# fcogidi/X3D-tf

Measured on AMD Instinct MI355X. Metric: clips/sec (fwd+bwd) X3D-M 16x224^2; depthwise HBM GB/s, higher is better.
Workload: dtype bf16

## Files before the change

### x3d-tf_amd/csrc/pw_bwd_wst.hip

```cpp
#include <stdlib.h>

#include "pw_gemm_ws.h"

struct PwBwdWstArgs {
  const void* g; const void* yraw; const float* coef;
  const void* wp; int wp_rows;
  void* dx;
  const void* braw; const float* b_ss; const float* egate; double* nc_sums;
  float* dw;
  int N, Co, Ci;
  long long P;
  int tiles_per_block;
  BnBwdFold fold;
  float* slab;
  int hot;
  int noflush;
};

#define BW_YRP 40

template <typename H, int NW, int KS, int CT>
__global__ __launch_bounds__(512, 2) void pw_bwd_wst_kernel(const PwBwdWstArgs a) {
  typedef typename HV<H>::x8 hx8;
  extern __shared__ __attribute__((aligned(16))) unsigned char smem_raw[];
  typedef H T;
  constexpr int BN = 32, OP = WS_OP, NT = 512, Kp = KS * 16, WP = Kp + 8, CoP = CT * 32, YRP = BW_YRP;
  static_assert(CoP >= Kp, "the row-read copy covers every staged dY row");
  constexpr int NSV = (Kp * 4 + NT - 1) / NT;
  H* Yt = (H*)smem_raw;
  H* Yr = (H*)(smem_raw + (size_t)2 * Kp * 64);
  H* Xh = (H*)(smem_raw + (size_t)2 * Kp * 64 + (size_t)2 * CoP * YRP * 2);
  float* Cs = (float*)(smem_raw + (size_t)2 * Kp * 64 + (size_t)2 * CoP * YRP * 2 + (size_t)NW * 32 * YRP * 2);
  float* Os = Cs + Kp * 4;
  const int tid = threadIdx.x, lane = tid & 63, wid = tid >> 6;
  const int r = lane & 31, half = lane >> 5;
  const int mt = (a.Ci + 31) >> 5;
  const int tiles_per_n = (int)((a.P + BN - 1) / BN);
  const int total_tiles = tiles_per_n * a.N;
  const int tile_begin = blockIdx.x * a.tiles_per_block;
  const int tile_end = min(tile_begin + a.tiles_per_block, total_tiles);
  if (tile_begin >= tile_end) return;
  float* myOs = Os + wid * 32 * OP;
  const int rb = blockIdx.y * NW + wid;
  const bool mw = wid < NW && rb < mt;

  {
    hx8 z;
#pragma unroll
    for (int e = 0; e < 8; e++) z[e] = (H)0.f;
    for (int i = tid; i < 2 * CoP * YRP / 8; i += NT) ((hx8*)Yr)[i] = z;
    for (int k = tid; k < Kp; k += NT) {
      f32x4 c = {0.f, 0.f, 0.f, 0.f};
      if (k < a.Co) {
        float cA_, cB_, cC_;
        bn_bwd_coef_load(a.coef, a.fold, k, blockIdx.x == 0 && blockIdx.y == 0, cA_, cB_, cC_);
        c[0] = cA_; c[1] = cB_; c[2] = cC_;
      }
      *(f32x4*)&Cs[k * 4] = c;
    }
  }

  hx8 A[KS];
  if (mw) {
    const H* wt = (const H*)a.wp + (long long)a.wp_rows * WP + ((long long)rb * KS * 64 + lane) * 8;
#pragma unroll
    for (int ks = 0; ks < KS; ks++) A[ks] = *(const hx8*)(wt + ks * 512);
  } else {
#pragma unroll
    for (int ks = 0; ks < KS; ks++)
#pragma unroll
      for (int e = 0; e < 8; e++) A[ks][e] = (H)0.f;
  }

  hx8 g0[NSV], y0[NSV], g1[NSV], y1[NSV];
  auto issue_loads = [&](int tile_, hx8 (&gr)[NSV], hx8 (&yr)[NSV]) {
    const int tile = a.hot ? tile_begin : min(tile_, tile_end - 1);
    const int n = tile / tiles_per_n;
    const long long p0 = (long long)(tile - n * tiles_per_n) * BN;
#pragma unroll
    for (int i = 0; i < NSV; i++) {
      const int v = tid + i * NT;
      const int k = v >> 2;
      const long long p = p0 + (v & 3) * 8;
      const bool ok = k < a.Co && p < a.P;
      const long long o = ok ? ((long long)n * a.Co + k) * a.P + p : 0;
      gr[i] = *(const hx8*)((const T*)a.g + o);
      yr[i] = *(const hx8*)((const T*)a.yraw + o);
    }
  };
  auto commit = [&](int tile, int buf, const hx8 (&gr)[NSV], const hx8 (&yr)[NSV]) {
    const int n = tile / tiles_per_n;
    const long long p0 = (long long)(tile - n * tiles_per_n) * BN;
#pragma unroll
    for (int i = 0; i < NSV; i++) {
      const int v = tid + i * NT;
      const int k = v >> 2;
      if (k >= Kp) continue;
      const bool ok = k < a.Co && p0 + (v & 3) * 8 < a.P;
      const f32x4 cf = *(const f32x4*)&Cs[k * 4];
      float val[8];
#pragma unroll
      for (int e = 0; e < 8; e++) val[e] = ok ? cf[0] * (float)gr[i][e] + cf[1] * (float)yr[i][e] + cf[2] : 0.f;
      hx8 hv;
#pragma unroll
      for (int e = 0; e < 8; e++) hv[e] = (H)val[e];
      *(hx8*)&Yt[(buf * Kp + k) * BN + (v & 3) * 8] = hv;
      *(hx8*)&Yr[(buf * CoP + k) * YRP + (v & 3) * 8] = hv;
    }
  };

  const int row = lane >> 1, c0 = 16 * (lane & 1);
  const int m = rb * 32 + row;
  const bool mrow = mw && m < a.Ci;
  hx8 eb0[2], eb1[2];
  float gl0, gl1;
  const float* gsrc = a.egate ? a.egate : a.b_ss;
  auto issue_braw = [&](int tile_, hx8 (&eb)[2], float& gl) {
    const int tile = a.hot ? tile_begin : min(tile_, tile_end - 1);
    const int n = tile / tiles_per_n;
    const long long p0 = (long long)(tile - n * tiles_per_n) * BN;
    gl = gsrc[(a.egate && mrow) ? (long long)n * a.Ci + m : 0];
#pragma unroll
    for (int hv = 0; hv < 2; hv++) {
      const long long p = p0 + c0 + 8 * hv;
      const long long o = (mrow && p < a.P) ? ((long long)n * a.Ci + m) * a.P + p : 0;
      eb[hv] = *(const hx8*)((const T*)a.braw + o);
    }
  };

  float st1 = 0.f, st2 = 0.f;
  auto flush_sums = [&](int n) {
    const float s1 = st1 + dpp_get<0xB1, 0xF>(st1), s2 = st2 + dpp_get<0xB1, 0xF>(st2);
    if (mrow && (lane & 1) == 0) {
      double* d = a.nc_sums + ((long long)n * a.Ci + m) * 2;
      atomic_add_d(d, (double)s1);
      atomic_add_d(d + 1, (double)s2);
    }
    st1 = 0.f;
    st2 = 0.f;
  };
  const float sb = mrow ? a.b_ss[m * 2] : 0.f, tb = mrow ? a.b_ss[m * 2 + 1] : 0.f;

  f32x16 acc_dw[CT];
#pragma unroll
  for (int s = 0; s < CT; s++)
#pragma unroll
    for (int e = 0; e < 16; e++) acc_dw[s][e] = 0.f;

  const int g16 = lane >> 4, q = (lane & 15) >> 2, pp = lane & 3;
  const int tr_off = (8 * (g16 >> 1) + q) * BN + 16 * (g16 & 1) + 4 * pp;
  typedef s16x4 __attribute__((address_space(3))) * lds_s16x4_ptr;

  int n_prev = tile_begin / tiles_per_n;
  issue_loads(tile_begin, g0, y0);
  issue_braw(tile_begin, eb0, gl0);
  __syncthreads();
  commit(tile_begin, 0, g0, y0);
  __syncthreads();
  issue_loads(tile_begin + 1, g1, y1);
  issue_loads(tile_begin + 2, g0, y0);

  typedef __attribute__((ext_vector_type(4))) unsigned int u32x4_;
  auto step = [&](int tile, int cur, hx8 (&gr)[NSV], hx8 (&yr)[NSV], hx8 (&eb)[2], float gl, hx8 (&ebn)[2], float& gln) {
    const int n = tile / tiles_per_n;
    const long long p0 = (long long)(tile - n * tiles_per_n) * BN;
    if (n != n_prev) flush_sums(n_prev);
    n_prev = n;
    issue_braw(tile + 1, ebn, gln);
    const float gt = (mrow && a.egate) ? gl : 1.0f;
    __amdgpu_buffer_rsrc_t dxr = __builtin_amdgcn_make_buffer_rsrc((T*)a.dx + (long long)n * a.Ci * a.P, 0,
                                                                   (int)((long long)a.Ci * a.P * 2), 0x00020000);

    f32x16 acc;
#pragma unroll
    for (int e = 0; e < 16; e++) acc[e] = 0.f;
    if (mw) {
      const H* xb = Yt + cur * (Kp * BN) + tr_off;
#pragma unroll
      for (int ks = 0; ks < KS; ks++) {
        const s16x4 b0 = __builtin_amdgcn_ds_read_tr16_b64_v4i16((lds_s16x4_ptr)(xb + ks * 16 * BN));
        const s16x4 b1 = __builtin_amdgcn_ds_read_tr16_b64_v4i16((lds_s16x4_ptr)(xb + (ks * 16 + 4) * BN));
        const s16x8 bs = {b0[0], b0[1], b0[2], b0[3], b1[0], b1[1], b1[2], b1[3]};
        acc = mfma16<H>(A[ks], __builtin_bit_cast(hx8, bs), acc);
      }
    }

    if (tile + 1 < tile_end) commit(tile + 1, cur ^ 1, gr, yr);

    if (mw) {
#pragma unroll
      for (int e = 0; e < 16; e++) myOs[((e & 3) + 8 * (e >> 2) + 4 * half) * OP + r] = acc[e];
#pragma unroll
      for (int hv = 0; hv < 2; hv++) {
        const long long p = p0 + c0 + 8 * hv;
        const bool ok = mrow && p < a.P;
        float val[8];
        {
          const f32x4 v0 = *(const f32x4*)&myOs[row * OP + c0 + 8 * hv], v1 = *(const f32x4*)&myOs[row * OP + c0 + 8 * hv + 4];
#pragma unroll
          for (int e = 0; e < 4; e++) { val[e] = v0[e]; val[4 + e] = v1[e]; }
        }
        hx8 xh;
        const SwishCoef sc_ = swish_coef(sb, tb, gt);
#pragma unroll
        for (int e = 0; e < 8; e++) {
          const float b = (float)eb[hv][e];
          float xs, d_;
          swish_bwd_(sc_, b, xs, d_);
          xh[e] = ok ? (H)xs : (H)0.f;
          const float dv = val[e] * d_;
          val[e] = dv;
          if (ok) { st1 += dv; st2 += dv * b; }
        }
        *(hx8*)&Xh[(wid * 32 + row) * YRP + c0 + 8 * hv] = xh;
        hx8 ov;
#pragma unroll
        for (int e = 0; e < 8; e++) ov[e] = (H)val[e];
        __builtin_amdgcn_raw_buffer_store_b128(__builtin_bit_cast(u32x4_, ov), dxr,
                                               ok ? (unsigned)(((long long)m * a.P + p) * 2) : 0x80000000u, 0, 0);
      }
      const H* yrow = Yr + (cur * CoP + r) * YRP + 8 * half;
      const H* xrow = Xh + (wid * 32 + r) * YRP + 8 * half;
#pragma unroll
      for (int ks = 0; ks < BN / 16; ks++) {
        const hx8 bf = *(const hx8*)(xrow + ks * 16);
#pragma unroll
        for (int s = 0; s < CT; s++) {
          const hx8 af = *(const hx8*)(yrow + s * 32 * YRP + ks * 16);
          acc_dw[s] = mfma16<H>(af, bf, acc_dw[s]);
        }
      }
    }
    __syncthreads();
    issue_loads(tile + 3, gr, yr);
  };
  for (int tile = tile_begin; tile < tile_end; tile += 2) {
    step(tile, 0, g1, y1, eb0, gl0, eb1, gl1);
    if (tile + 1 < tile_end) step(tile + 1, 1, g0, y0, eb1, gl1, eb0, gl0);
  }
  flush_sums(n_prev);

  if (mw && !a.noflush) {
    const int ci = rb * 32 + r;
    float* slab = a.slab ? a.slab + (long long)blockIdx.x * a.Co * a.Ci : nullptr;
#pragma unroll
    for (int s = 0; s < CT; s++)
#pragma unroll
      for (int e = 0; e < 16; e++) {
        const int co = s * 32 + (e & 3) + 8 * (e >> 2) + 4 * half;
        if (co < a.Co && ci < a.Ci) {
          if (slab) slab[(long long)co * a.Ci + ci] = acc_dw[s][e];
          else atomicAdd(&a.dw[(long long)co * a.Ci + ci], acc_dw[s][e]);
        }
      }
  }
}

template <int NW, int KS, int CT>
static inline size_t bw_lds_bytes() {
  return (size_t)2 * KS * 16 * 64 + (size_t)2 * CT * 32 * BW_YRP * 2 + (size_t)NW * 32 * BW_YRP * 2 + (size_t)KS * 16 * 16 +
         (size_t)NW * 32 * WS_OP * 4;
}

bool pw_bwd_wst_applies(const x3d_pw_bwd_args* b) {
  if (x3d_env_int("X3D_PW_BWD_WST", 1) == 0) return false;
  if (!x3d_is_half(b->dtype) || !b->w_panel || (!b->coef && !b->coef_fold) || !b->yraw || b->epi != X3D_EPI_SWISH_BWD || b->tail_c) return false;
  const int ks = (b->Cout + 15) >> 4;
  if (!((b->Cin > 128 && b->Cin <= 224 && ks == 6) || (b->Cin > 224 && b->Cin <= 448 && ks == 12 && x3d_env_int("X3D_PW_BWD_WST5", 1) != 0))) return false;
  const long long P = (long long)b->T * b->H * b->W;
  if (P % 8 || P >= (1ll << 31) || (long long)b->Cin * P * 2 >= (1ll << 31)) return false;
  const void* ps[] = {b->g, b->yraw, b->dx, b->w_panel, b->braw};
  for (const void* p : ps) if (!p || ((uintptr_t)p % 16)) return false;
  return true;
}

static inline void bw_grid(int N, long long P, int Ci, long long* tpb, long long* gx, int* slices) {
  *slices = ceil_div(ceil_div(Ci, 32), 7);
  x3d_persistent_grid(ceil_div_ll(P, 32) * N, x3d_device_cus() / *slices, tpb, gx);
}

template <typename H, int KS, int CT>
static int bw_launch(PwBwdWstArgs& a, hipStream_t st) {
  constexpr int NW = 7;
  const size_t lds = bw_lds_bytes<NW, KS, CT>();
  X3D_DESCRIBE("pw_bwd_wst_kernel<%s, %d, %d, %d>", HV<H>::name, NW, KS, CT);
  auto kern = pw_bwd_wst_kernel<H, NW, KS, CT>;
  static bool attr_set = false;
  if (!attr_set) {
    (void)hipFuncSetAttribute((const void*)kern, hipFuncAttributeMaxDynamicSharedMemorySize, 128 * 1024);
    attr_set = true;
  }
  const long long total_tiles = ceil_div_ll(a.P, 32) * a.N;
  X3D_REQUIRE(total_tiles < (1ll << 31), "pw_bwd_wst: too many tiles");
  long long tpb, gx;
  int slices;
  bw_grid(a.N, a.P, a.Ci, &tpb, &gx, &slices);
  a.tiles_per_block = (int)tpb;
  a.noflush = x3d_env_int("X3D_PW_BWD_NOFLUSH", 0);
  a.hot = x3d_env_int("X3D_PW_BWD_HOT", 0);
  hipLaunchKernelGGL(kern, dim3((unsigned)gx, (unsigned)slices), dim3(512), lds, st, a);
  X3D_LAUNCH_CHECK("pw_bwd_wst");
  return X3D_OK;
}

int pw_bwd_wst(const x3d_pw_bwd_args* b, hipStream_t st) {
  X3D_REQUIRE(b->braw && b->b_scale_shift && b->nc_sums, "pw_bwd: SWISH_BWD needs braw/b_scale_shift/nc_sums");
  PwBwdWstArgs a;
  memset(&a, 0, sizeof(a));
  a.g = b->g; a.yraw = b->yraw; a.coef = b->coef;
  a.wp = b->w_panel; a.wp_rows = (b->Cin + 31) & ~31;
  a.dx = b->dx; a.braw = b->braw; a.b_ss = b->b_scale_shift; a.egate = b->gate; a.nc_sums = b->nc_sums;
  a.dw = b->dw; a.slab = b->dw_slab; a.fold = bn_bwd_fold_arg(b->coef_fold);
  a.N = b->N; a.Co = b->Cout; a.Ci = b->Cin;
  a.P = (long long)b->T * b->H * b->W;
  if (((b->Cout + 15) >> 4) == 12) return b->dtype == X3D_F16 ? bw_launch<f16, 12, 6>(a, st) : bw_launch<bf16, 12, 6>(a, st);
  return b->dtype == X3D_F16 ? bw_launch<f16, 6, 3>(a, st) : bw_launch<bf16, 6, 3>(a, st);
}

int pw_bwd_wst_dw_parts(const x3d_pw_bwd_args* b) {
  long long tpb, gx;
  int slices;
  bw_grid(b->N, (long long)b->T * b->H * b->W, b->Cin, &tpb, &gx, &slices);
  return (int)gx;
}
```

### x3d-tf_amd/csrc/pw_bwd_wsta.hip

```cpp
#include <stdlib.h>

#include "pw_gemm_ws.h"

struct PwBwdWstaArgs {
  const void* g; const void* yraw; const float* coef;
  const void* wp; int wp_rows;
  void* dx;
  const void* add;
  const void* x;
  float* dw;
  const void* tail_c; const void* tail_r; double* tail_sums_c; double* tail_sums_r;
  int N, Co, Ci;
  long long P;
  int tiles_per_block;
  BnBwdFold fold;
  float* slab;
  int hot;
  int noflush;
};

#define BWA_RP 40

template <typename H, int NW, int KS, int CT, int TAIL>
__global__ __launch_bounds__(512, 2) void pw_bwd_wsta_kernel(const PwBwdWstaArgs a) {
  typedef typename HV<H>::x8 hx8;
  extern __shared__ __attribute__((aligned(16))) unsigned char smem_raw[];
  typedef H T;
  constexpr int BN = 32, OP = WS_OP, NT = 512, Kp = KS * 16, WP = Kp + 8, CoP = CT * 32, CiP = NW * 32, RP = BWA_RP;
  static_assert(CoP >= Kp && CT <= 8, "dY rows / weight-gradient waves");
  constexpr int NSV = (Kp * 4 + NT - 1) / NT;
  constexpr size_t YT_B = (size_t)2 * Kp * 64, YR_B = (size_t)2 * CoP * RP * 2, XR_B = (size_t)2 * CiP * RP * 2;
  H* Yt = (H*)smem_raw;
  H* Yr = (H*)(smem_raw + YT_B);
  H* Xr = (H*)(smem_raw + YT_B + YR_B);
  float* Cs = (float*)(smem_raw + YT_B + YR_B + XR_B);
  float* Os = Cs + Kp * 4;
  const int tid = threadIdx.x, lane = tid & 63, wid = tid >> 6;
  const int r = lane & 31, half = lane >> 5;
  const int tiles_per_n = (int)((a.P + BN - 1) / BN);
  const int total_tiles = tiles_per_n * a.N;
  const int tile_begin = blockIdx.x * a.tiles_per_block;
  const int tile_end = min(tile_begin + a.tiles_per_block, total_tiles);
  if (tile_begin >= tile_end) return;
  float* myOs = Os + (wid < NW ? wid : 0) * 32 * OP;
  const bool xw = wid < NW && wid * 32 < a.Ci;
  const bool ww = wid < CT && wid * 32 < a.Co;

  {
    hx8 z;
#pragma unroll
    for (int e = 0; e < 8; e++) z[e] = (H)0.f;
    for (int i = tid; i < (int)((YR_B + XR_B) / 16); i += NT) ((hx8*)Yr)[i] = z;
    for (int k = tid; k < Kp; k += NT) {
      f32x4 c = {0.f, 0.f, 0.f, 0.f};
      if (k < a.Co) {
        float cA_, cB_, cC_;
        bn_bwd_coef_load(a.coef, a.fold, k, blockIdx.x == 0 && blockIdx.y == 0, cA_, cB_, cC_);
        c[0] = cA_; c[1] = cB_; c[2] = cC_;
      }
      *(f32x4*)&Cs[k * 4] = c;
    }
  }

  hx8 A[KS];
  if (xw) {
    const H* wt = (const H*)a.wp + (long long)a.wp_rows * WP + ((long long)wid * KS * 64 + lane) * 8;
#pragma unroll
    for (int ks = 0; ks < KS; ks++) A[ks] = *(const hx8*)(wt + ks * 512);
  } else {
#pragma unroll
    for (int ks = 0; ks < KS; ks++)
#pragma unroll
      for (int e = 0; e < 8; e++) A[ks][e] = (H)0.f;
  }

  hx8 g0[NSV], y0[NSV], g1[NSV], y1[NSV], x0, x1;
  auto issue_loads = [&](int tile_, hx8 (&gr)[NSV], hx8 (&yr)[NSV], hx8& xr) __attribute__((always_inline)) {
    const int tile = a.hot ? tile_begin : min(tile_, tile_end - 1);
    const int n = tile / tiles_per_n;
    const long long p0 = (long long)(tile - n * tiles_per_n) * BN;
#pragma unroll
    for (int i = 0; i < NSV; i++) {
      const int v = tid + i * NT;
      const int k = v >> 2;
      const long long p = p0 + (v & 3) * 8;
      const long long o = (k < a.Co && p < a.P) ? ((long long)n * a.Co + k) * a.P + p : 0;
      gr[i] = *(const hx8*)((const T*)a.g + o);
      yr[i] = *(const hx8*)((const T*)a.yraw + o);
    }
    {
      const int mrow = tid >> 2;
      const long long p = p0 + (tid & 3) * 8;
      const long long o = (mrow < a.Ci && p < a.P) ? ((long long)n * a.Ci + mrow) * a.P + p : 0;
      xr = *(const hx8*)((const T*)a.x + o);
    }
  };
  auto commit = [&](int tile, int buf, const hx8 (&gr)[NSV], const hx8 (&yr)[NSV], const hx8& xr) __attribute__((always_inline)) {
    const int n = tile / tiles_per_n;
    const long long p0 = (long long)(tile - n * tiles_per_n) * BN;
#pragma unroll
    for (int i = 0; i < NSV; i++) {
      const int v = tid + i * NT;
      const int k = v >> 2;
      if (k >= Kp) continue;
      const bool ok = k < a.Co && p0 + (v & 3) * 8 < a.P;
      const f32x4 cf = *(const f32x4*)&Cs[k * 4];
      hx8 hv;
#pragma unroll
      for (int e = 0; e < 8; e++) hv[e] = (H)(ok ? cf[0] * (float)gr[i][e] + cf[1] * (float)yr[i][e] + cf[2] : 0.f);
      *(hx8*)&Yt[(buf * Kp + k) * BN + (v & 3) * 8] = hv;
      *(hx8*)&Yr[(buf * CoP + k) * RP + (v & 3) * 8] = hv;
    }
    const int mrow = tid >> 2;
    if (mrow < CiP) {
      const bool ok = mrow < a.Ci && p0 + (tid & 3) * 8 < a.P;
      hx8 hv = xr;
      if (!ok) {
#pragma unroll
        for (int e = 0; e < 8; e++) hv[e] = (H)0.f;
      }
      *(hx8*)&Xr[(buf * CiP + mrow) * RP + (tid & 3) * 8] = hv;
    }
  };

  const int row = lane >> 1, c0 = 16 * (lane & 1);
  const int m = wid * 32 + row;
  const bool mrow_ok = xw && m < a.Ci;
  constexpr int NEO = 1 + (TAIL >= 1) + (TAIL == 2);
  hx8 eo0[NEO][2], eo1[NEO][2];
  auto issue_epi = [&](int tile_, hx8 (&eo)[NEO][2]) __attribute__((always_inline)) {
    const int tile = a.hot ? tile_begin : min(tile_, tile_end - 1);
    const int n = tile / tiles_per_n;
    const long long p0 = (long long)(tile - n * tiles_per_n) * BN;
#pragma unroll
    for (int hv = 0; hv < 2; hv++) {
      const long long p = p0 + c0 + 8 * hv;
      const long long o = (mrow_ok && p < a.P) ? ((long long)n * a.Ci + m) * a.P + p : 0;
      eo[0][hv] = *(const hx8*)((const T*)a.add + o);
      if constexpr (TAIL >= 1) eo[1][hv] = *(const hx8*)((const T*)a.tail_c + o);
      if constexpr (TAIL == 2) eo[2][hv] = *(const hx8*)((const T*)a.tail_r + o);
    }
  };
  float tg = 0.f, tgc = 0.f, tgr = 0.f;

  f32x16 acc_dw[NW];
#pragma unroll
  for (int s = 0; s < NW; s++)
#pragma unroll
    for (int e = 0; e < 16; e++) acc_dw[s][e] = 0.f;

  const int g16 = lane >> 4, q = (lane & 15) >> 2, pp = lane & 3;
  const int tr_off = (8 * (g16 >> 1) + q) * BN + 16 * (g16 & 1) + 4 * pp;
  typedef s16x4 __attribute__((address_space(3))) * lds_s16x4_ptr;
  typedef __attribute__((ext_vector_type(4))) unsigned int u32x4_;

  issue_loads(tile_begin, g0, y0, x0);
  issue_epi(tile_begin, eo0);
  __syncthreads();
  commit(tile_begin, 0, g0, y0, x0);
  __syncthreads();
  issue_loads(tile_begin + 1, g1, y1, x1);
  issue_loads(tile_begin + 2, g0, y0, x0);

  auto step = [&](int tile, int cur, hx8 (&gr)[NSV], hx8 (&yr)[NSV], hx8& xr, hx8 (&eo)[NEO][2], hx8 (&eon)[NEO][2])
      __attribute__((always_inline)) {
    const int n = tile / tiles_per_n;
    const long long p0 = (long long)(tile - n * tiles_per_n) * BN;
    issue_epi(tile + 1, eon);
    __amdgpu_buffer_rsrc_t dxr = __builtin_amdgcn_make_buffer_rsrc((T*)a.dx + (long long)n * a.Ci * a.P, 0,
                                                                   (int)((long long)a.Ci * a.P * 2), 0x00020000);
    f32x16 acc;
#pragma unroll
    for (int e = 0; e < 16; e++) acc[e] = 0.f;
    if (xw) {
      const H* xb = Yt + cur * (Kp * BN) + tr_off;
#pragma unroll
      for (int ks = 0; ks < KS; ks++) {
        const s16x4 b0 = __builtin_amdgcn_ds_read_tr16_b64_v4i16((lds_s16x4_ptr)(xb + ks * 16 * BN));
        const s16x4 b1 = __builtin_amdgcn_ds_read_tr16_b64_v4i16((lds_s16x4_ptr)(xb + (ks * 16 + 4) * BN));
        const s16x8 bs = {b0[0], b0[1], b0[2], b0[3], b1[0], b1[1], b1[2], b1[3]};
        acc = mfma16<H>(A[ks], __builtin_bit_cast(hx8, bs), acc);
      }
    }
    if (ww) {
      const H* yrow = Yr + (cur * CoP + wid * 32 + r) * RP + 8 * half;
      const H* xrow = Xr + (cur * CiP + r) * RP + 8 * half;
#pragma unroll
      for (int ks = 0; ks < BN / 16; ks++) {
        const hx8 af = *(const hx8*)(yrow + ks * 16);
#pragma unroll
        for (int s = 0; s < NW; s++) {
          const hx8 bf = *(const hx8*)(xrow + s * 32 * RP + ks * 16);
          acc_dw[s] = mfma16<H>(af, bf, acc_dw[s]);
        }
      }
    }
    if (tile + 1 < tile_end) commit(tile + 1, cur ^ 1, gr, yr, xr);

    if (xw) {
#pragma unroll
      for (int e = 0; e < 16; e++) myOs[((e & 3) + 8 * (e >> 2) + 4 * half) * OP + r] = acc[e];
#pragma unroll
      for (int hv = 0; hv < 2; hv++) {
        const long long p = p0 + c0 + 8 * hv;
        const bool ok = mrow_ok && p < a.P;
        float val[8];
        {
          const f32x4 v0 = *(const f32x4*)&myOs[row * OP + c0 + 8 * hv], v1 = *(const f32x4*)&myOs[row * OP + c0 + 8 * hv + 4];
#pragma unroll
          for (int e = 0; e < 4; e++) { val[e] = v0[e]; val[4 + e] = v1[e]; }
        }
#pragma unroll
        for (int e = 0; e < 8; e++) val[e] += (float)eo[0][hv][e];
        if constexpr (TAIL >= 1) {
          const hx8 xv = *(const hx8*)&Xr[(cur * CiP + m) * RP + c0 + 8 * hv];
#pragma unroll
          for (int e = 0; e < 8; e++) {
            const float gm = (ok && (float)xv[e] > 0.f) ? round_to<T>(val[e]) : 0.f;
            val[e] = gm;
            tg += gm;
            tgc += gm * (float)eo[1][hv][e];
            if constexpr (TAIL == 2) tgr += gm * (float)eo[2][hv][e];
          }
        }
        hx8 ov;
#pragma unroll
        for (int e = 0; e < 8; e++) ov[e] = (H)val[e];
        __builtin_amdgcn_raw_buffer_store_b128(__builtin_bit_cast(u32x4_, ov), dxr,
                                               ok ? (unsigned)(((long long)m * a.P + p) * 2) : 0x80000000u, 0, 0);
      }
    }
    __syncthreads();
    issue_loads(tile + 3, gr, yr, xr);
  };
  for (int tile = tile_begin; tile < tile_end; tile += 2) {
    step(tile, 0, g1, y1, x1, eo0, eo1);
    if (tile + 1 < tile_end) step(tile + 1, 1, g0, y0, x0, eo1, eo0);
  }

  if constexpr (TAIL >= 1) {
    const float s0 = tg + dpp_get<0xB1, 0xF>(tg), s1 = tgc + dpp_get<0xB1, 0xF>(tgc);
    float s2 = 0.f;
    if constexpr (TAIL == 2) s2 = tgr + dpp_get<0xB1, 0xF>(tgr);
    if (mrow_ok && (lane & 1) == 0) {
      atomic_add_d(&a.tail_sums_c[m * 2], (double)s0);
      atomic_add_d(&a.tail_sums_c[m * 2 + 1], (double)s1);
      if constexpr (TAIL == 2) {
        atomic_add_d(&a.tail_sums_r[m * 2], (double)s0);
        atomic_add_d(&a.tail_sums_r[m * 2 + 1], (double)s2);
      }
    }
  }
  if (ww && !a.noflush) {
    float* slab = a.slab ? a.slab + (long long)blockIdx.x * a.Co * a.Ci : nullptr;
#pragma unroll
    for (int s = 0; s < NW; s++) {
      const int ci = s * 32 + r;
#pragma unroll
      for (int e = 0; e < 16; e++) {
        const int co = wid * 32 + (e & 3) + 8 * (e >> 2) + 4 * half;
        if (co < a.Co && ci < a.Ci) {
          if (slab) slab[(long long)co * a.Ci + ci] = acc_dw[s][e];
          else atomicAdd(&a.dw[(long long)co * a.Ci + ci], acc_dw[s][e]);
        }
      }
    }
  }
}

template <int NW, int KS, int CT>
static inline size_t bwa_lds_bytes() {
  return (size_t)2 * KS * 16 * 64 + (size_t)2 * CT * 32 * BWA_RP * 2 + (size_t)2 * NW * 32 * BWA_RP * 2 + (size_t)KS * 16 * 16 +
         (size_t)NW * 32 * WS_OP * 4;
}

bool pw_bwd_wsta_applies(const x3d_pw_bwd_args* b) {
  if (x3d_env_int("X3D_PW_BWD_WSTA", 1) == 0) return false;
  if (!x3d_is_half(b->dtype) || !b->w_panel || (!b->coef && !b->coef_fold) || !b->yraw || b->epi != X3D_EPI_ADD || !b->x || !b->add) return false;
  if (b->Cin <= 64 || b->Cin > 96 || ((b->Cout + 15) >> 4) != 14) return false;
  const long long P = (long long)b->T * b->H * b->W;
  if (P % 8 || P >= (1ll << 31) || (long long)b->Cin * P * 2 >= (1ll << 31)) return false;
  const void* ps[] = {b->g, b->yraw, b->dx, b->w_panel, b->x, b->add};
  for (const void* p : ps) if (!p || ((uintptr_t)p % 16)) return false;
  if (b->tail_r) return false;
  if (b->tail_c && ((uintptr_t)b->tail_c % 16)) return false;
  return true;
}

template <typename H, int TAIL>
static int bwa_launch(PwBwdWstaArgs& a, hipStream_t st) {
  constexpr int NW = 3, KS = 14, CT = 7;
  const size_t lds = bwa_lds_bytes<NW, KS, CT>();
  X3D_DESCRIBE("pw_bwd_wsta_kernel<%s, %d, %d, %d, %d>", HV<H>::name, NW, KS, CT, TAIL);
  auto kern = pw_bwd_wsta_kernel<H, NW, KS, CT, TAIL>;
  static bool attr_set = false;
  if (!attr_set) {
    (void)hipFuncSetAttribute((const void*)kern, hipFuncAttributeMaxDynamicSharedMemorySize, 128 * 1024);
    attr_set = true;
  }
  const long long total_tiles = ceil_div_ll(a.P, 32) * a.N;
  X3D_REQUIRE(total_tiles < (1ll << 31), "pw_bwd_wsta: too many tiles");
  long long tpb, gx;
  x3d_persistent_grid(total_tiles, x3d_device_cus(), &tpb, &gx);
  a.tiles_per_block = (int)tpb;
  a.noflush = x3d_env_int("X3D_PW_BWD_NOFLUSH", 0);
  a.hot = x3d_env_int("X3D_PW_BWD_HOT", 0);
  hipLaunchKernelGGL(kern, dim3((unsigned)gx), dim3(512), lds, st, a);
  X3D_LAUNCH_CHECK("pw_bwd_wsta");
  return X3D_OK;
}

int pw_bwd_wsta(const x3d_pw_bwd_args* b, hipStream_t st) {
  X3D_REQUIRE(!b->tail_c || x3d_describe.out || (b->tail_sums_c && (!b->tail_r || b->tail_sums_r)), "pw_bwd: tail_c / tail_r need their sums");
  PwBwdWstaArgs a;
  memset(&a, 0, sizeof(a));
  a.g = b->g; a.yraw = b->yraw; a.coef = b->coef;
  a.wp = b->w_panel; a.wp_rows = (b->Cin + 31) & ~31;
  a.dx = b->dx; a.add = b->add; a.x = b->x; a.dw = b->dw; a.slab = b->dw_slab; a.fold = bn_bwd_fold_arg(b->coef_fold);
  a.tail_c = b->tail_c; a.tail_r = b->tail_r; a.tail_sums_c = b->tail_sums_c; a.tail_sums_r = b->tail_sums_r;
  a.N = b->N; a.Co = b->Cout; a.Ci = b->Cin;
  a.P = (long long)b->T * b->H * b->W;
  const bool tail = b->tail_c != nullptr;
  if (b->dtype == X3D_F16) return tail ? bwa_launch<f16, 1>(a, st) : bwa_launch<f16, 0>(a, st);
  return tail ? bwa_launch<bf16, 1>(a, st) : bwa_launch<bf16, 0>(a, st);
}

int pw_bwd_wsta_dw_parts(const x3d_pw_bwd_args* b) {
  long long tpb, gx;
  x3d_persistent_grid(ceil_div_ll((long long)b->T * b->H * b->W, 32) * b->N, x3d_device_cus(), &tpb, &gx);
  return (int)gx;
}
```

### x3d-tf_amd/csrc/pw_gemm_ws.h

```cpp
#pragma once
#include <type_traits>

#include "pw_gemm_bf16.h"

#define WS_BN 32
#define WS_G 8
#define WS_OP 36
#define WS_MAXMT 4
#ifndef WS_OCC
#define WS_OCC 2
#endif

template <typename H, int PRO, int EPI>
__global__ __launch_bounds__(256, WS_OCC) void pw_gemm_ws_kernel(const PwGemmArgs a) {
  typedef typename HV<H>::x8 hx8; typedef typename HV<H>::x4 hx4; typedef typename HV<H>::x2 hx2;
  extern __shared__ __attribute__((aligned(16))) unsigned char smem_raw[];
  typedef H T;
  constexpr int BN = WS_BN, G = WS_G, OP = WS_OP;
  constexpr bool HAS_SUMS = (EPI == EPI_STATS) || (EPI == X3D_EPI_SWISH_BWD);
  constexpr int CSW = (PRO == PRO_AFFINE) ? 2 : 4;
  constexpr int NSV = 7;
  const int Kp = a.KC, WP = Kp + 8;
  const int ksteps = Kp / 16;
  H* Xs = (H*)smem_raw;
  float* Cs = (float*)(smem_raw + (size_t)Kp * 64);
  float* Os = (float*)(smem_raw + (size_t)Kp * 64 + (size_t)Kp * 16);
  const int tid = threadIdx.x, lane = tid & 63, wid = tid >> 6;
  const int r = lane & 31, half = lane >> 5;
  const int mt = (a.M + 31) >> 5;
  const int tiles_per_n = (int)((a.P + BN - 1) / BN);
  const int total_tiles = tiles_per_n * a.N;
  const int tile_begin = blockIdx.x * a.tiles_per_block;
  const int tile_end = min(tile_begin + a.tiles_per_block, total_tiles);
  float* myOs = Os + wid * 32 * OP;

  auto fill_coef = [&](int n) {
    if constexpr (PRO != PRO_NONE) {
      for (int k = tid; k < Kp; k += 256) {
        f32x4 c = {0.f, 0.f, 0.f, 0.f};
        if (k < a.K) {
          if constexpr (PRO == PRO_AFFINE) {
            const float g = a.gate ? a.gate[(long long)n * a.K + k] : 1.0f;
            c[0] = a.coef[k * 2] * g;
            c[1] = a.coef[k * 2 + 1] * g;
          } else {
            c[0] = a.coef[k * 4]; c[1] = a.coef[k * 4 + 1]; c[2] = a.coef[k * 4 + 2];
          }
        }
        if constexpr (CSW == 2) *(float2*)&Cs[k * 2] = make_float2(c[0], c[1]);
        else *(f32x4*)&Cs[k * 4] = c;
      }
    }
  };
  if (tile_begin < tile_end) fill_coef(tile_begin / tiles_per_n);

  hx8 xr[NSV], yr[PRO == PRO_BNBWD ? NSV : 1];
  auto issue_loads = [&](int tile) {
    const int n = tile / tiles_per_n;
    const long long p0 = (long long)(tile - n * tiles_per_n) * BN;
#pragma unroll
    for (int i = 0; i < NSV; i++) {
      const int v = tid + i * 256;
      const int k = v >> 2;
      const long long p = p0 + (v & 3) * 8;
      hx8 z;
#pragma unroll
      for (int e = 0; e < 8; e++) z[e] = (H)0.f;
      xr[i] = z;
      if constexpr (PRO == PRO_BNBWD) yr[i] = z;
      if (k < a.K && p < a.P) {
        const long long o = ((long long)n * a.K + k) * a.Pin + p;
        xr[i] = *(const hx8*)((const T*)a.x + o);
        if constexpr (PRO == PRO_BNBWD) yr[i] = *(const hx8*)((const T*)a.x2 + o);
      }
    }
  };
  auto commit = [&]() {
#pragma unroll
    for (int i = 0; i < NSV; i++) {
      const int v = tid + i * 256;
      const int k = v >> 2;
      if (k >= Kp) continue;
      H* dst = &Xs[k * BN + (v & 3) * 8];
      if constexpr (PRO == PRO_NONE) {
        *(hx8*)dst = xr[i];
      } else {
        float val[8];
#pragma unroll
        for (int e = 0; e < 8; e++) val[e] = (float)xr[i][e];
        if constexpr (PRO == PRO_AFFINE) {
          const float2 cf = *(const float2*)&Cs[k * 2];
#pragma unroll
          for (int e = 0; e < 8; e++) val[e] = cf.x * val[e] + cf.y;
          act_vec<8>(val, a.act);
        } else {
          const f32x4 cf = *(const f32x4*)&Cs[k * 4];
#pragma unroll
          for (int e = 0; e < 8; e++) val[e] = cf[0] * val[e] + cf[1] * (float)yr[i][e] + cf[2];
        }
        VecIO<H, 8>::store(dst, val);
      }
    }
  };

  float st1[HAS_SUMS ? WS_MAXMT : 1], st2[HAS_SUMS ? WS_MAXMT : 1];
  if constexpr (HAS_SUMS) {
#pragma unroll
    for (int i = 0; i < WS_MAXMT; i++) { st1[i] = 0.f; st2[i] = 0.f; }
  }
  auto flush_sums = [&](int n) {
    if constexpr (HAS_SUMS) {
#pragma unroll
      for (int i = 0; i < WS_MAXMT; i++) {
        const int mi = wid + 4 * i;
        const float s1 = st1[i] + dpp_get<0xB1, 0xF>(st1[i]), s2 = st2[i] + dpp_get<0xB1, 0xF>(st2[i]);
        const int m = mi * 32 + (lane >> 1);
        if (mi < mt && (lane & 1) == 0 && m < a.M) {
          if constexpr (EPI == EPI_STATS) {
            if (a.stats) {
              double* sp = stats_replica(a.stats, a.M, blockIdx.x);
              atomic_add_d(&sp[m * 2], (double)s1);
              atomic_add_d(&sp[m * 2 + 1], (double)s2);
            }
          } else {
            double* d = a.nc_sums + ((long long)n * a.M + m) * 2;
            atomic_add_d(d, (double)s1);
            atomic_add_d(d + 1, (double)s2);
          }
        }
        st1[i] = 0.f;
        st2[i] = 0.f;
      }
    }
  };

  const int g16 = lane >> 4, q = (lane & 15) >> 2, pp = lane & 3;
  const int tr_row = 8 * (g16 >> 1) + q;
  const int tr_col = 16 * (g16 & 1) + 4 * pp;
  typedef s16x4 __attribute__((address_space(3))) * lds_s16x4_ptr;

  if (tile_begin < tile_end) issue_loads(tile_begin);
  int n_prev = tile_begin < tile_end ? tile_begin / tiles_per_n : 0;
  for (int tile = tile_begin; tile < tile_end; ++tile) {
    const int n = tile / tiles_per_n;
    const long long p0 = (long long)(tile - n * tiles_per_n) * BN;
    if (n != n_prev) {
      if constexpr (EPI == X3D_EPI_SWISH_BWD) flush_sums(n_prev);
      if constexpr (PRO == PRO_AFFINE) { if (a.gate) fill_coef(n); }
    }
    n_prev = n;
    __syncthreads();
    commit();
    __syncthreads();
    if (tile + 1 < tile_end) issue_loads(tile + 1);

    for (int i = 0; i < WS_MAXMT; i++) {
      const int mi = wid + 4 * i;
      if (mi >= mt) break;
      const H* wrow = (const H*)a.wp + (long long)a.wp_rows * WP + ((long long)mi * ksteps * 64 + lane) * 8;
      f32x16 acc;
#pragma unroll
      for (int j = 0; j < 16; j++) acc[j] = 0.f;
      hx8 A0[G], A1[G];
      auto loadA = [&](hx8 (&A)[G], int ks0, auto FULL) {
#pragma unroll
        for (int j = 0; j < G; j++) {
          if constexpr (decltype(FULL)::value) {
            A[j] = *(const hx8*)(wrow + (ks0 + j) * 512);
          } else {
            hx8 z;
#pragma unroll
            for (int e = 0; e < 8; e++) z[e] = (H)0.f;
            A[j] = (ks0 + j < ksteps) ? *(const hx8*)(wrow + (ks0 + j) * 512) : z;
          }
        }
      };
      auto mmaA = [&](const hx8 (&A)[G], int ks0, auto FULL) {
#pragma unroll
        for (int j = 0; j < G; j++) {
          if (decltype(FULL)::value || ks0 + j < ksteps) {
            const int kk = (ks0 + j) * 16;
            const s16x4 b0 = __builtin_amdgcn_ds_read_tr16_b64_v4i16((lds_s16x4_ptr)(&Xs[(kk + tr_row) * BN + tr_col]));
            const s16x4 b1 = __builtin_amdgcn_ds_read_tr16_b64_v4i16((lds_s16x4_ptr)(&Xs[(kk + tr_row + 4) * BN + tr_col]));
            const s16x8 bs = {b0[0], b0[1], b0[2], b0[3], b1[0], b1[1], b1[2], b1[3]};
            acc = mfma16<H>(A[j], __builtin_bit_cast(hx8, bs), acc);
          }
        }
      };
      auto load_g = [&](hx8 (&A)[G], int ks0) {
        if (ks0 + G <= ksteps) loadA(A, ks0, std::true_type{});
        else if (ks0 < ksteps) loadA(A, ks0, std::false_type{});
      };
      auto mma_g = [&](const hx8 (&A)[G], int ks0) {
        if (ks0 + G <= ksteps) mmaA(A, ks0, std::true_type{});
        else if (ks0 < ksteps) mmaA(A, ks0, std::false_type{});
      };
      load_g(A0, 0);
      for (int ks0 = 0; ks0 < ksteps; ks0 += 2 * G) {
        load_g(A1, ks0 + G);
        mma_g(A0, ks0);
        load_g(A0, ks0 + 2 * G);
        mma_g(A1, ks0 + G);
      }

#pragma unroll
      for (int j = 0; j < 16; j++) myOs[((j & 3) + 8 * (j >> 2) + 4 * half) * OP + r] = acc[j];
      const int row = lane >> 1, c0 = 16 * (lane & 1);
      const int m = mi * 32 + row;
      if (m < a.M) {
        float sb = 0.f, tb = 0.f, gt = 1.f;
        if constexpr (EPI == X3D_EPI_SWISH_BWD) {
          sb = a.b_ss[m * 2]; tb = a.b_ss[m * 2 + 1];
          gt = a.egate ? a.egate[(long long)n * a.M + m] : 1.0f;
        }
        if constexpr (EPI == EPI_BNADD) bnadd_coef(a, m, true, sb, tb, gt);
#pragma unroll
        for (int hv = 0; hv < 2; hv++) {
          const long long p = p0 + c0 + 8 * hv;
          if (p >= a.P) continue;
          const long long o = ((long long)n * a.M + m) * a.P + p;
          float val[8];
          {
            const f32x4 v0 = *(const f32x4*)&myOs[row * OP + c0 + 8 * hv], v1 = *(const f32x4*)&myOs[row * OP + c0 + 8 * hv + 4];
#pragma unroll
            for (int e = 0; e < 4; e++) { val[e] = v0[e]; val[4 + e] = v1[e]; }
          }
          if constexpr (EPI == X3D_EPI_ADD) {
            float ad[8];
            VecIO<T, 8>::load((const T*)a.add + o, ad);
#pragma unroll
            for (int e = 0; e < 8; e++) val[e] += ad[e];
          } else if constexpr (EPI == EPI_BNADD) {
            float ad[8];
#pragma unroll
            for (int e = 0; e < 8; e++) ad[e] = 0.f;
            if (a.add) VecIO<T, 8>::load((const T*)a.add + o, ad);
            const float lo = a.eact == X3D_ACT_RELU ? 0.f : -__builtin_inff();
#pragma unroll
            for (int e = 0; e < 8; e++) val[e] = fmaxf(sb * val[e] + tb + gt * ad[e], lo);
          } else if constexpr (EPI == X3D_EPI_SWISH_BWD) {
            float b[8];
            VecIO<T, 8>::load((const T*)a.braw + o, b);
            const SwishCoef sc_ = swish_coef(sb, tb, gt);
#pragma unroll
            for (int e = 0; e < 8; e++) {
              float xh_, d_;
              swish_bwd_(sc_, b[e], xh_, d_);
              const float dv = val[e] * d_;
              val[e] = dv;
              st1[i] += dv;
              st2[i] += dv * b[e];
            }
          }
          if constexpr (EPI == EPI_STATS) {
#pragma unroll
            for (int e = 0; e < 8; e++) { st1[i] += val[e]; st2[i] += val[e] * val[e]; }
          }
          VecIO<T, 8>::store((T*)a.y + o, val);
        }
      }
    }
  }
  if (tile_begin < tile_end) flush_sums(n_prev);
}

static inline size_t pw_ws_lds_bytes(int K) {
  const int Kp = (K + 15) & ~15;
  return (size_t)Kp * 64 + (size_t)Kp * 16 + (size_t)4 * 32 * WS_OP * 4;
}

static inline bool pw_ws_applies(const PwGemmArgs& a, int vec, int ovec) {
  const int e_ws = x3d_env_int("X3D_PW_WS", -1);
  if (e_ws == 0) return false;
  if (!a.wp || vec < 8 || ovec < 8 || a.stride != 1 || (a.P % 8) != 0) return false;
  if (a.K > 448 || a.M > 128 * WS_MAXMT) return false;
  if (e_ws == 1) return true;
  const long long tiles128 = ceil_div_ll(a.P, 128) * a.N;
  return tiles128 <= 1024 && a.K >= 320 && a.M <= 256;
}

template <typename H, int PRO, int EPI>
static int pw_ws_launch(PwGemmArgs& a, hipStream_t st) {
  a.KC = (a.K + 15) & ~15;
  const size_t lds = pw_ws_lds_bytes(a.K);
  X3D_DESCRIBE("pw_gemm_ws_kernel<%s, %d, %d>", HV<H>::name, PRO, EPI);
  auto kern = pw_gemm_ws_kernel<H, PRO, EPI>;
  static bool attr_set = false;
  if (!attr_set) {
    (void)hipFuncSetAttribute((const void*)kern, hipFuncAttributeMaxDynamicSharedMemorySize, 96 * 1024);
    attr_set = true;
  }
  static size_t occ_lds[8];
  static int occ_slots[8], occ_n = 0;
  int slots = 0;
  for (int i = 0; i < occ_n; i++) if (occ_lds[i] == lds) slots = occ_slots[i];
  if (slots == 0) {
    int nb = 0, dev = 0, cus = 256;
    hipDeviceProp_t prop;
    if (hipGetDevice(&dev) == hipSuccess && hipGetDeviceProperties(&prop, dev) == hipSuccess) cus = prop.multiProcessorCount;
    if (hipOccupancyMaxActiveBlocksPerMultiprocessor(&nb, kern, 256, lds) != hipSuccess || nb < 1) nb = 1;
    slots = nb * cus;
    if (occ_n < 8) { occ_lds[occ_n] = lds; occ_slots[occ_n] = slots; occ_n++; }
  }
  const long long total_tiles = ceil_div_ll(a.P, WS_BN) * a.N;
  X3D_REQUIRE(total_tiles < (1ll << 31), "pw_gemm_ws: too many tiles");
  long long tpb = ceil_div_ll(total_tiles, slots);
  if (tpb < 2) tpb = 2;
  a.tiles_per_block = (int)tpb;
  const long long gx = ceil_div_ll(total_tiles, tpb);
  hipLaunchKernelGGL(kern, dim3((unsigned)gx), dim3(256), lds, st, a);
  X3D_LAUNCH_CHECK("pw_gemm_ws");
  return X3D_OK;
}
```

Baseline: 3224.

## Drop duplicate row-major dY copy and swizzle the shared tile for both reads

The backward pointwise kernels used to stage each dY tile twice in LDS: once for the transposed-read dX GEMM and once padded for the row-read dW GEMM. Now they stage a single XOR-swizzled copy that both GEMMs read, using matching swizzled offsets for the transposed loads and the row loads. This removes the second LDS store per element, the zero-init pass and a sizeable chunk of LDS, which may allow higher occupancy. It also adds optional cycle-counter stamp instrumentation, compiled out by default. The risk is bank conflicts if the swizzle does not suit both access patterns, and the CoP==Kp assert now rules out other configurations.

```diff
diff --git a/x3d-tf_amd/csrc/pw_bwd_wst.hip b/x3d-tf_amd/csrc/pw_bwd_wst.hip
--- a/x3d-tf_amd/csrc/pw_bwd_wst.hip
+++ b/x3d-tf_amd/csrc/pw_bwd_wst.hip
@@ -17,6 +17,15 @@
   int noflush;
 };
 
+#ifdef BWS_STAMPS
+__device__ unsigned long long bw_stamps[2][64];
+#define BW_STAMP(i) do { if (threadIdx.x == 0 && blockIdx.y == 0 && (blockIdx.x == 0 || blockIdx.x == gridDim.x - 1) && (i) < 64) bw_stamps[blockIdx.x == 0 ? 0 : 1][i] = __builtin_readcyclecounter(); } while (0)
+extern "C" int x3d_debug_bw_stamps(unsigned long long* out) { return hipMemcpyFromSymbol(out, HIP_SYMBOL(bw_stamps), sizeof(bw_stamps)) == hipSuccess ? 0 : 1; }
+#else
+#define BW_STAMP(i) do { } while (0)
+#endif
+#define BWS_STEP_STAMPS 11
+
 #define BW_YRP 40
 
 template <typename H, int NW, int KS, int CT>
@@ -25,12 +34,11 @@
   extern __shared__ __attribute__((aligned(16))) unsigned char smem_raw[];
   typedef H T;
   constexpr int BN = 32, OP = WS_OP, NT = 512, Kp = KS * 16, WP = Kp + 8, CoP = CT * 32, YRP = BW_YRP;
-  static_assert(CoP >= Kp, "the row-read copy covers every staged dY row");
+  static_assert(CoP == Kp, "the dW row blocks read exactly the staged dY rows (commit() writes all Kp of them)");
   constexpr int NSV = (Kp * 4 + NT - 1) / NT;
   H* Yt = (H*)smem_raw;
-  H* Yr = (H*)(smem_raw + (size_t)2 * Kp * 64);
-  H* Xh = (H*)(smem_raw + (size_t)2 * Kp * 64 + (size_t)2 * CoP * YRP * 2);
-  float* Cs = (float*)(smem_raw + (size_t)2 * Kp * 64 + (size_t)2 * CoP * YRP * 2 + (size_t)NW * 32 * YRP * 2);
+  H* Xh = (H*)(smem_raw + (size_t)2 * Kp * 64);
+  float* Cs = (float*)(smem_raw + (size_t)2 * Kp * 64 + (size_t)NW * 32 * YRP * 2);
   float* Os = Cs + Kp * 4;
   const int tid = threadIdx.x, lane = tid & 63, wid = tid >> 6;
   const int r = lane & 31, half = lane >> 5;
@@ -40,15 +48,12 @@
   const int tile_begin = blockIdx.x * a.tiles_per_block;
   const int tile_end = min(tile_begin + a.tiles_per_block, total_tiles);
   if (tile_begin >= tile_end) return;
+  BW_STAMP(0);
   float* myOs = Os + wid * 32 * OP;
   const int rb = blockIdx.y * NW + wid;
   const bool mw = wid < NW && rb < mt;
 
   {
-    hx8 z;
-#pragma unroll
-    for (int e = 0; e < 8; e++) z[e] = (H)0.f;
-    for (int i = tid; i < 2 * CoP * YRP / 8; i += NT) ((hx8*)Yr)[i] = z;
     for (int k = tid; k < Kp; k += NT) {
       f32x4 c = {0.f, 0.f, 0.f, 0.f};
       if (k < a.Co) {
@@ -104,8 +109,7 @@
       hx8 hv;
 #pragma unroll
       for (int e = 0; e < 8; e++) hv[e] = (H)val[e];
-      *(hx8*)&Yt[(buf * Kp + k) * BN + (v & 3) * 8] = hv;
-      *(hx8*)&Yr[(buf * CoP + k) * YRP + (v & 3) * 8] = hv;
+      *(hx8*)&Yt[(buf * Kp + k) * BN + ws_swz(k, v & 3) * 8] = hv;
     }
   };
 
@@ -148,15 +152,19 @@
     for (int e = 0; e < 16; e++) acc_dw[s][e] = 0.f;
 
   const int g16 = lane >> 4, q = (lane & 15) >> 2, pp = lane & 3;
-  const int tr_off = (8 * (g16 >> 1) + q) * BN + 16 * (g16 & 1) + 4 * pp;
+  const int tr_row = (8 * (g16 >> 1) + q) * BN, tr_u = 2 * (g16 & 1) + (pp >> 1), tr_e = 4 * (pp & 1);
+  const int tr_off0 = tr_row + (tr_u ^ (2 * half)) * 8 + tr_e, tr_off1 = tr_row + 4 * BN + (tr_u ^ (2 * half + 1)) * 8 + tr_e;
   typedef s16x4 __attribute__((address_space(3))) * lds_s16x4_ptr;
 
   int n_prev = tile_begin / tiles_per_n;
   issue_loads(tile_begin, g0, y0);
   issue_braw(tile_begin, eb0, gl0);
+  BW_STAMP(1);
   __syncthreads();
+  BW_STAMP(2);
   commit(tile_begin, 0, g0, y0);
   __syncthreads();
+  BW_STAMP(3);
   issue_loads(tile_begin + 1, g1, y1);
   issue_loads(tile_begin + 2, g0, y0);
 
@@ -164,6 +172,7 @@
   auto step = [&](int tile, int cur, hx8 (&gr)[NSV], hx8 (&yr)[NSV], hx8 (&eb)[2], float gl, hx8 (&ebn)[2], float& gln) {
     const int n = tile / tiles_per_n;
     const long long p0 = (long long)(tile - n * tiles_per_n) * BN;
+    const int sj = tile - tile_begin < BWS_STEP_STAMPS ? 4 + 5 * (tile - tile_begin) : 64;
     if (n != n_prev) flush_sums(n_prev);
     n_prev = n;
     issue_braw(tile + 1, ebn, gln);
@@ -175,17 +184,19 @@
 #pragma unroll
     for (int e = 0; e < 16; e++) acc[e] = 0.f;
     if (mw) {
-      const H* xb = Yt + cur * (Kp * BN) + tr_off;
+      const H* xb = Yt + cur * (Kp * BN);
 #pragma unroll
       for (int ks = 0; ks < KS; ks++) {
-        const s16x4 b0 = __builtin_amdgcn_ds_read_tr16_b64_v4i16((lds_s16x4_ptr)(xb + ks * 16 * BN));
-        const s16x4 b1 = __builtin_amdgcn_ds_read_tr16_b64_v4i16((lds_s16x4_ptr)(xb + (ks * 16 + 4) * BN));
+        const s16x4 b0 = __builtin_amdgcn_ds_read_tr16_b64_v4i16((lds_s16x4_ptr)(xb + tr_off0 + ks * 16 * BN));
+        const s16x4 b1 = __builtin_amdgcn_ds_read_tr16_b64_v4i16((lds_s16x4_ptr)(xb + tr_off1 + ks * 16 * BN));
         const s16x8 bs = {b0[0], b0[1], b0[2], b0[3], b1[0], b1[1], b1[2], b1[3]};
         acc = mfma16<H>(A[ks], __builtin_bit_cast(hx8, bs), acc);
       }
     }
 
+    BW_STAMP(sj);
     if (tile + 1 < tile_end) commit(tile + 1, cur ^ 1, gr, yr);
+    BW_STAMP(sj + 1);
 
     if (mw) {
 #pragma unroll
@@ -219,25 +230,30 @@
         __builtin_amdgcn_raw_buffer_store_b128(__builtin_bit_cast(u32x4_, ov), dxr,
                                                ok ? (unsigned)(((long long)m * a.P + p) * 2) : 0x80000000u, 0, 0);
       }
-      const H* yrow = Yr + (cur * CoP + r) * YRP + 8 * half;
+      BW_STAMP(sj + 2);
+      const H* yrow = Yt + (cur * Kp + r) * BN;
       const H* xrow = Xh + (wid * 32 + r) * YRP + 8 * half;
 #pragma unroll
       for (int ks = 0; ks < BN / 16; ks++) {
         const hx8 bf = *(const hx8*)(xrow + ks * 16);
 #pragma unroll
         for (int s = 0; s < CT; s++) {
-          const hx8 af = *(const hx8*)(yrow + s * 32 * YRP + ks * 16);
+          const hx8 af = *(const hx8*)(yrow + s * 32 * BN + ws_swz(r, 2 * ks + half) * 8);
           acc_dw[s] = mfma16<H>(af, bf, acc_dw[s]);
         }
       }
     }
+    BW_STAMP(sj + 3);
     __syncthreads();
+    BW_STAMP(sj + 4);
     issue_loads(tile + 3, gr, yr);
   };
   for (int tile = tile_begin; tile < tile_end; tile += 2) {
     step(tile, 0, g1, y1, eb0, gl0, eb1, gl1);
-    if (tile + 1 < tile_end) step(tile + 1, 1, g0, y0, eb1, gl1, eb0, gl0);
-  }
+    if (tile + 1 >= tile_end) break;
+    step(tile + 1, 1, g0, y0, eb1, gl1, eb0, gl0);
+  }
+  BW_STAMP(60);
   flush_sums(n_prev);
 
   if (mw && !a.noflush) {
@@ -254,11 +270,12 @@
         }
       }
   }
+  BW_STAMP(61);
 }
 
 template <int NW, int KS, int CT>
 static inline size_t bw_lds_bytes() {
-  return (size_t)2 * KS * 16 * 64 + (size_t)2 * CT * 32 * BW_YRP * 2 + (size_t)NW * 32 * BW_YRP * 2 + (size_t)KS * 16 * 16 +
+  return (size_t)2 * KS * 16 * 64 + (size_t)NW * 32 * BW_YRP * 2 + (size_t)KS * 16 * 16 +
          (size_t)NW * 32 * WS_OP * 4;
 }
 
diff --git a/x3d-tf_amd/csrc/pw_bwd_wsta.hip b/x3d-tf_amd/csrc/pw_bwd_wsta.hip
--- a/x3d-tf_amd/csrc/pw_bwd_wsta.hip
+++ b/x3d-tf_amd/csrc/pw_bwd_wsta.hip
@@ -19,6 +19,15 @@
   int noflush;
 };
 
+#ifdef BWS_STAMPS
+__device__ unsigned long long bwa_stamps[2][64];
+#define BWA_STAMP(i) do { if (threadIdx.x == 0 && (blockIdx.x == 0 || blockIdx.x == gridDim.x - 1) && (i) < 64) bwa_stamps[blockIdx.x == 0 ? 0 : 1][i] = __builtin_readcyclecounter(); } while (0)
+extern "C" int x3d_debug_bwa_stamps(unsigned long long* out) { return hipMemcpyFromSymbol(out, HIP_SYMBOL(bwa_stamps), sizeof(bwa_stamps)) == hipSuccess ? 0 : 1; }
+#else
+#define BWA_STAMP(i) do { } while (0)
+#endif
+#define BWS_STEP_STAMPS 11
+
 #define BWA_RP 40
 
 template <typename H, int NW, int KS, int CT, int TAIL>
@@ -27,13 +36,12 @@
   extern __shared__ __attribute__((aligned(16))) unsigned char smem_raw[];
   typedef H T;
   constexpr int BN = 32, OP = WS_OP, NT = 512, Kp = KS * 16, WP = Kp + 8, CoP = CT * 32, CiP = NW * 32, RP = BWA_RP;
-  static_assert(CoP >= Kp && CT <= 8, "dY rows / weight-gradient waves");
+  static_assert(CoP == Kp && CT <= 8, "the dW row blocks read exactly the staged dY rows (commit() writes all Kp of them) / weight-gradient waves");
   constexpr int NSV = (Kp * 4 + NT - 1) / NT;
-  constexpr size_t YT_B = (size_t)2 * Kp * 64, YR_B = (size_t)2 * CoP * RP * 2, XR_B = (size_t)2 * CiP * RP * 2;
+  constexpr size_t YT_B = (size_t)2 * Kp * 64, XR_B = (size_t)2 * CiP * RP * 2;
   H* Yt = (H*)smem_raw;
-  H* Yr = (H*)(smem_raw + YT_B);
-  H* Xr = (H*)(smem_raw + YT_B + YR_B);
-  float* Cs = (float*)(smem_raw + YT_B + YR_B + XR_B);
+  H* Xr = (H*)(smem_raw + YT_B);
+  float* Cs = (float*)(smem_raw + YT_B + XR_B);
   float* Os = Cs + Kp * 4;
   const int tid = threadIdx.x, lane = tid & 63, wid = tid >> 6;
   const int r = lane & 31, half = lane >> 5;
@@ -42,15 +50,12 @@
   const int tile_begin = blockIdx.x * a.tiles_per_block;
   const int tile_end = min(tile_begin + a.tiles_per_block, total_tiles);
   if (tile_begin >= tile_end) return;
+  BWA_STAMP(0);
   float* myOs = Os + (wid < NW ? wid : 0) * 32 * OP;
   const bool xw = wid < NW && wid * 32 < a.Ci;
   const bool ww = wid < CT && wid * 32 < a.Co;
 
   {
-    hx8 z;
-#pragma unroll
-    for (int e = 0; e < 8; e++) z[e] = (H)0.f;
-    for (int i = tid; i < (int)((YR_B + XR_B) / 16); i += NT) ((hx8*)Yr)[i] = z;
     for (int k = tid; k < Kp; k += NT) {
       f32x4 c = {0.f, 0.f, 0.f, 0.f};
       if (k < a.Co) {
@@ -108,8 +113,7 @@
       hx8 hv;
 #pragma unroll
       for (int e = 0; e < 8; e++) hv[e] = (H)(ok ? cf[0] * (float)gr[i][e] + cf[1] * (float)yr[i][e] + cf[2] : 0.f);
-      *(hx8*)&Yt[(buf * Kp + k) * BN + (v & 3) * 8] = hv;
-      *(hx8*)&Yr[(buf * CoP + k) * RP + (v & 3) * 8] = hv;
+      *(hx8*)&Yt[(buf * Kp + k) * BN + ws_swz(k, v & 3) * 8] = hv;
     }
     const int mrow = tid >> 2;
     if (mrow < CiP) {
@@ -150,15 +154,19 @@
     for (int e = 0; e < 16; e++) acc_dw[s][e] = 0.f;
 
   const int g16 = lane >> 4, q = (lane & 15) >> 2, pp = lane & 3;
-  const int tr_off = (8 * (g16 >> 1) + q) * BN + 16 * (g16 & 1) + 4 * pp;
+  const int tr_row = (8 * (g16 >> 1) + q) * BN, tr_u = 2 * (g16 & 1) + (pp >> 1), tr_e = 4 * (pp & 1);
+  const int tr_off0 = tr_row + (tr_u ^ (2 * half)) * 8 + tr_e, tr_off1 = tr_row + 4 * BN + (tr_u ^ (2 * half + 1)) * 8 + tr_e;
   typedef s16x4 __attribute__((address_space(3))) * lds_s16x4_ptr;
   typedef __attribute__((ext_vector_type(4))) unsigned int u32x4_;
 
   issue_loads(tile_begin, g0, y0, x0);
   issue_epi(tile_begin, eo0);
+  BWA_STAMP(1);
   __syncthreads();
+  BWA_STAMP(2);
   commit(tile_begin, 0, g0, y0, x0);
   __syncthreads();
+  BWA_STAMP(3);
   issue_loads(tile_begin + 1, g1, y1, x1);
   issue_loads(tile_begin + 2, g0, y0, x0);
 
@@ -166,6 +174,7 @@
       __attribute__((always_inline)) {
     const int n = tile / tiles_per_n;
     const long long p0 = (long long)(tile - n * tiles_per_n) * BN;
+    const int sj = tile - tile_begin < BWS_STEP_STAMPS ? 4 + 5 * (tile - tile_begin) : 64;
     issue_epi(tile + 1, eon);
     __amdgpu_buffer_rsrc_t dxr = __builtin_amdgcn_make_buffer_rsrc((T*)a.dx + (long long)n * a.Ci * a.P, 0,
                                                                    (int)((long long)a.Ci * a.P * 2), 0x00020000);
@@ -173,21 +182,22 @@
 #pragma unroll
     for (int e = 0; e < 16; e++) acc[e] = 0.f;
     if (xw) {
-      const H* xb = Yt + cur * (Kp * BN) + tr_off;
+      const H* xb = Yt + cur * (Kp * BN);
 #pragma unroll
       for (int ks = 0; ks < KS; ks++) {
-        const s16x4 b0 = __builtin_amdgcn_ds_read_tr16_b64_v4i16((lds_s16x4_ptr)(xb + ks * 16 * BN));
-        const s16x4 b1 = __builtin_amdgcn_ds_read_tr16_b64_v4i16((lds_s16x4_ptr)(xb + (ks * 16 + 4) * BN));
+        const s16x4 b0 = __builtin_amdgcn_ds_read_tr16_b64_v4i16((lds_s16x4_ptr)(xb + tr_off0 + ks * 16 * BN));
+        const s16x4 b1 = __builtin_amdgcn_ds_read_tr16_b64_v4i16((lds_s16x4_ptr)(xb + tr_off1 + ks * 16 * BN));
         const s16x8 bs = {b0[0], b0[1], b0[2], b0[3], b1[0], b1[1], b1[2], b1[3]};
         acc = mfma16<H>(A[ks], __builtin_bit_cast(hx8, bs), acc);
       }
     }
+    BWA_STAMP(sj);
     if (ww) {
-      const H* yrow = Yr + (cur * CoP + wid * 32 + r) * RP + 8 * half;
+      const H* yrow = Yt + (cur * Kp + wid * 32 + r) * BN;
       const H* xrow = Xr + (cur * CiP + r) * RP + 8 * half;
 #pragma unroll
       for (int ks = 0; ks < BN / 16; ks++) {
-        const hx8 af = *(const hx8*)(yrow + ks * 16);
+        const hx8 af = *(const hx8*)(yrow + ws_swz(r, 2 * ks + half) * 8);
 #pragma unroll
         for (int s = 0; s < NW; s++) {
           const hx8 bf = *(const hx8*)(xrow + s * 32 * RP + ks * 16);
@@ -195,7 +205,9 @@
         }
       }
     }
+    BWA_STAMP(sj + 1);
     if (tile + 1 < tile_end) commit(tile + 1, cur ^ 1, gr, yr, xr);
+    BWA_STAMP(sj + 2);
 
     if (xw) {
 #pragma unroll
@@ -230,7 +242,9 @@
                                                ok ? (unsigned)(((long long)m * a.P + p) * 2) : 0x80000000u, 0, 0);
       }
     }
+    BWA_STAMP(sj + 3);
     __syncthreads();
+    BWA_STAMP(sj + 4);
     issue_loads(tile + 3, gr, yr, xr);
   };
   for (int tile = tile_begin; tile < tile_end; tile += 2) {
@@ -238,6 +252,7 @@
     if (tile + 1 < tile_end) step(tile + 1, 1, g0, y0, x0, eo1, eo0);
   }
 
+  BWA_STAMP(60);
   if constexpr (TAIL >= 1) {
     const float s0 = tg + dpp_get<0xB1, 0xF>(tg), s1 = tgc + dpp_get<0xB1, 0xF>(tgc);
     float s2 = 0.f;
@@ -266,11 +281,12 @@
       }
     }
   }
+  BWA_STAMP(61);
 }
 
 template <int NW, int KS, int CT>
 static inline size_t bwa_lds_bytes() {
-  return (size_t)2 * KS * 16 * 64 + (size_t)2 * CT * 32 * BWA_RP * 2 + (size_t)2 * NW * 32 * BWA_RP * 2 + (size_t)KS * 16 * 16 +
+  return (size_t)2 * KS * 16 * 64 + (size_t)2 * NW * 32 * BWA_RP * 2 + (size_t)KS * 16 * 16 +
          (size_t)NW * 32 * WS_OP * 4;
 }
 
diff --git a/x3d-tf_amd/csrc/pw_gemm_ws.h b/x3d-tf_amd/csrc/pw_gemm_ws.h
--- a/x3d-tf_amd/csrc/pw_gemm_ws.h
+++ b/x3d-tf_amd/csrc/pw_gemm_ws.h
@@ -10,6 +10,8 @@
 #ifndef WS_OCC
 #define WS_OCC 2
 #endif
+
+__device__ __forceinline__ int ws_swz(int row, int unit) { return unit ^ ((row >> 2) & 3); }
 
 template <typename H, int PRO, int EPI>
 __global__ __launch_bounds__(256, WS_OCC) void pw_gemm_ws_kernel(const PwGemmArgs a) {
```

Result: no change. 3237, median of 6 (+0.4%).
